# lmb-freiburg/hand3d

Measured on NVIDIA H100. Metric: images/sec full pipeline 320x320, higher is better.
Workload: dtype bf16 hi/lo split x3 MMA passes, fp32 accumulate (fp32 parity, 1e-3)

## Files before the change

### hand3d_b200/csrc/conv_wgmma.cu

```cuda
#include <cuda.h>

#include <algorithm>
#include <cstdlib>
#include <cstring>
#include <vector>

#include "common.cuh"
#include "split_fmt.cuh"
#include "wgmma_common.cuh"

namespace h3d {

namespace {

constexpr int BM = 128;
constexpr int BK = 64;
constexpr int kThreads = 384;
constexpr int kConsumerThreads = 256;
constexpr int A_TILE_BYTES = BM * BK * 2;
constexpr int STG_COLS = 64;
constexpr int STG_PITCH = STG_COLS + 1;
constexpr int STG_BYTES = BM * STG_PITCH * 4;
constexpr int kSmemBudget = 227 * 1024 - 2048 - STG_BYTES;

__host__ __device__ constexpr int stage_bytes(int BN, int PASSES) { return (PASSES >= 3 ? 2 : 1) * (A_TILE_BYTES + BN * BK * 2); }
__host__ __device__ constexpr int num_stages(int BN, int PASSES) {
    return kSmemBudget / stage_bytes(BN, PASSES) > 8 ? 8 : kSmemBudget / stage_bytes(BN, PASSES);
}
__host__ __device__ constexpr int smem_bytes(int BN, int PASSES) { return num_stages(BN, PASSES) * stage_bytes(BN, PASSES) + STG_BYTES + 2048; }

struct TcParams {
    const float* bias;
    uint16_t* y_hi; uint16_t* y_lo; uint8_t* y_l8; uint8_t* y_h8; int Cy_total, cy_off;
    float corr_scale;
    float* yf; int Cyf_total, cyf_off;
    int B, H, W, k, pad, cin_chunks;
    int TW, TH, TB, tiles_w, tiles_h, n_tiles, num_tiles;
    int n_valid;
    int pool;
    int chunk_kb;
    int leaky;
    int* err_flag;
};

template <int PASSES, bool FP16>
__device__ __forceinline__ void epilogue_store32(const TcParams& p, const float* a, int64_t pix, int n, bool valid) {
    float f[32];
    const float4* bp = reinterpret_cast<const float4*>(p.bias + n);
#pragma unroll
    for (int q = 0; q < 8; ++q) {
        const float4 bv = __ldg(bp + q);
        if (PASSES == 4) {
            f[4 * q + 0] = fmaf(a[4 * q + 0], p.corr_scale, bv.x);
            f[4 * q + 1] = fmaf(a[4 * q + 1], p.corr_scale, bv.y);
            f[4 * q + 2] = fmaf(a[4 * q + 2], p.corr_scale, bv.z);
            f[4 * q + 3] = fmaf(a[4 * q + 3], p.corr_scale, bv.w);
        } else {
            f[4 * q + 0] = a[4 * q + 0] + bv.x;
            f[4 * q + 1] = a[4 * q + 1] + bv.y;
            f[4 * q + 2] = a[4 * q + 2] + bv.z;
            f[4 * q + 3] = a[4 * q + 3] + bv.w;
        }
    }
    if (p.leaky) {
#pragma unroll
        for (int q = 0; q < 32; ++q) f[q] = fmaxf(f[q], kNegSlope * f[q]);
    }
    if (p.pool == 1) {
#pragma unroll
        for (int q = 0; q < 32; ++q) {
            f[q] = fmaxf(f[q], __shfl_xor_sync(0xFFFFFFFFu, f[q], 1));
            f[q] = fmaxf(f[q], __shfl_xor_sync(0xFFFFFFFFu, f[q], p.TW));
        }
    }
    if (!valid) return;
    if (n + 32 > p.n_valid) {
        const int cnt = p.n_valid - n;
        if (p.yf && cnt > 0) {
            float* dst = p.yf + pix * p.Cyf_total + p.cyf_off + n;
#pragma unroll
            for (int q = 0; q < 32; ++q)
                if (q < cnt) dst[q] = f[q];
        }
#pragma unroll
        for (int q = 0; q < 32; ++q)
            if (q >= cnt) f[q] = 0.f;
    } else if (p.yf) {
        if (((p.Cyf_total | p.cyf_off) & 3) == 0) {
            float4* dst = reinterpret_cast<float4*>(p.yf + pix * p.Cyf_total + p.cyf_off + n);
#pragma unroll
            for (int q = 0; q < 8; ++q) dst[q] = make_float4(f[4 * q], f[4 * q + 1], f[4 * q + 2], f[4 * q + 3]);
        } else {
            float* dst = p.yf + pix * p.Cyf_total + p.cyf_off + n;
#pragma unroll
            for (int q = 0; q < 32; ++q) dst[q] = f[q];
        }
    }
    if (p.y_hi) {
        const int64_t off = pix * p.Cy_total + p.cy_off + n;
        uint4* dh = reinterpret_cast<uint4*>(p.y_hi + off);
        uint4* dl = reinterpret_cast<uint4*>(p.y_lo + off);
#pragma unroll
        for (int g = 0; g < 4; ++g) {
            uint32_t hi[4], lo[4];
#pragma unroll
            for (int q = 0; q < 4; ++q) {
                float x0 = f[8 * g + 2 * q], x1 = f[8 * g + 2 * q + 1];
                if (PASSES == 4) {
                    x0 = fminf(fmaxf(x0 * kF8XMainScale, -65504.f), 65504.f);
                    x1 = fminf(fmaxf(x1 * kF8XMainScale, -65504.f), 65504.f);
                }
                hi[q] = pack_hi2<FP16>(x0, x1);
                if (PASSES == 3) {
                    const float2 r = unpack2<FP16>(hi[q]);
                    lo[q] = pack_hi2<FP16>(x0 - r.x, x1 - r.y);
                }
            }
            dh[g] = make_uint4(hi[0], hi[1], hi[2], hi[3]);
            if (PASSES == 3 && p.y_lo) dl[g] = make_uint4(lo[0], lo[1], lo[2], lo[3]);
        }
        if (PASSES == 4) {
            uint32_t l8[8], h8[8];
#pragma unroll
            for (int q = 0; q < 8; ++q) {
                uint32_t wl = 0, wh = 0;
#pragma unroll
                for (int e = 0; e < 4; ++e) {
                    const F8cPlanes pl = f32_to_f8c(f[4 * q + e]);
                    wl |= (uint32_t)pl.l8 << (8 * e); wh |= (uint32_t)pl.h8 << (8 * e);
                }
                l8[q] = wl; h8[q] = wh;
            }
            uint4* d8l = reinterpret_cast<uint4*>(p.y_l8 + off);
            uint4* d8h = reinterpret_cast<uint4*>(p.y_h8 + off);
            d8l[0] = make_uint4(l8[0], l8[1], l8[2], l8[3]); d8l[1] = make_uint4(l8[4], l8[5], l8[6], l8[7]);
            d8h[0] = make_uint4(h8[0], h8[1], h8[2], h8[3]); d8h[1] = make_uint4(h8[4], h8[5], h8[6], h8[7]);
        }
    }
}

template <int BN, int PASSES>
struct RingCfg {
    static constexpr int STAGES = num_stages(BN, PASSES);
    static constexpr int STAGE_BYTES = stage_bytes(BN, PASSES);
    static constexpr int B_TILE_BYTES = BN * BK * 2;
    static constexpr int A8_TILE_BYTES = BM * BK, B8_TILE_BYTES = BN * BK;
    static_assert(STAGES >= 3, "the consumers hold two stages while the producer refills a third");
};

template <int BN, int PASSES>
__device__ __forceinline__ void produce_kblock(Ring& r, const CUtensorMap* x_hi, const CUtensorMap* x_lo, const CUtensorMap* x_h8,
                                               const CUtensorMap* w_hi, const CUtensorMap* w_lo, const CUtensorMap* w_l8,
                                               int a0, int a1, int a2, int a3, int kcol, int n0, int* err_flag) {
    using C = RingCfg<BN, PASSES>;
    mbar_wait(&r.empty[r.stage], r.phase ^ 1, err_flag, 1);
    if (elect_one()) {
        uint8_t* st = r.base + r.stage * C::STAGE_BYTES;
        uint64_t* fb = &r.full[r.stage];
        mbar_expect_tx(fb, C::STAGE_BYTES);
        tma_load_4d(x_hi, st, fb, a0, a1, a2, a3);
        tma_load_2d(w_hi, st + (PASSES >= 3 ? 2 : 1) * A_TILE_BYTES, fb, kcol, n0);
        if (PASSES == 3) {
            tma_load_4d(x_lo, st + A_TILE_BYTES, fb, a0, a1, a2, a3);
            tma_load_2d(w_lo, st + 2 * A_TILE_BYTES + C::B_TILE_BYTES, fb, kcol, n0);
        }
        if (PASSES == 4) {
            tma_load_4d(x_lo, st + A_TILE_BYTES, fb, a0, a1, a2, a3);
            tma_load_4d(x_h8, st + A_TILE_BYTES + C::A8_TILE_BYTES, fb, a0, a1, a2, a3);
            tma_load_2d(w_lo, st + 2 * A_TILE_BYTES + C::B_TILE_BYTES, fb, kcol, n0);
            tma_load_2d(w_l8, st + 2 * A_TILE_BYTES + C::B_TILE_BYTES + C::B8_TILE_BYTES, fb, kcol, n0);
        }
    }
    __syncwarp();
    if (++r.stage == C::STAGES) { r.stage = 0; r.phase ^= 1; }
}

template <int BN, int PASSES, bool FP16>
__device__ __forceinline__ void mma_tile(Ring& r, int kblocks, int chunk_kb, float* racc, int wg, int lane, int* err_flag) {
    using C = RingCfg<BN, PASSES>;
    constexpr int NR = BN / 2;
    constexpr int NR8 = PASSES == 4 ? NR : 1;
    float acc[NR], acc8[NR8];
#pragma unroll
    for (int i = 0; i < NR; ++i) acc[i] = 0.f;
#pragma unroll
    for (int i = 0; i < NR8; ++i) acc8[i] = 0.f;
    for (int kb0 = 0; kb0 < kblocks; kb0 += chunk_kb) {
        const int kb1 = min(kblocks, kb0 + chunk_kb);
        int pend = -1;
        for (int kb = kb0; kb < kb1; ++kb) {
            mbar_wait(&r.full[r.stage], r.phase, err_flag, 3);
            const uint32_t sa = smem_u32(r.base + r.stage * C::STAGE_BYTES);
            const uint32_t a_rows = (uint32_t)wg * 64 * 128;
            const uint64_t a_hi = desc_sw128(sa + a_rows);
            const uint64_t a_lo = desc_sw128(sa + A_TILE_BYTES + a_rows);
            const uint64_t b_hi = desc_sw128(sa + (PASSES >= 3 ? 2 : 1) * A_TILE_BYTES);
            const uint64_t b_lo = desc_sw128(sa + 2 * A_TILE_BYTES + C::B_TILE_BYTES);
            fence_regs<NR>(acc);
            fence_regs<NR8>(acc8);
            wgmma_fence();
#pragma unroll
            for (int j = 0; j < BK / 16; ++j) {
                const uint64_t koff = (uint64_t)j * 2;
                mma16<BN, FP16>(acc, a_hi + koff, b_hi + koff, (uint32_t)((kb > kb0) | (j != 0)));
                if (PASSES == 3) {
                    mma16<BN, FP16>(acc, a_hi + koff, b_lo + koff, 1u);
                    mma16<BN, FP16>(acc, a_lo + koff, b_hi + koff, 1u);
                }
            }
            if (PASSES == 4) {
                const uint32_t a8_rows = (uint32_t)wg * 64 * 64;
                const uint64_t a_l8 = desc_sw64(sa + A_TILE_BYTES + a8_rows);
                const uint64_t a_h8 = desc_sw64(sa + A_TILE_BYTES + C::A8_TILE_BYTES + a8_rows);
                const uint64_t b_h8 = desc_sw64(sa + 2 * A_TILE_BYTES + C::B_TILE_BYTES);
                const uint64_t b_l8 = desc_sw64(sa + 2 * A_TILE_BYTES + C::B_TILE_BYTES + C::B8_TILE_BYTES);
#pragma unroll
                for (int j = 0; j < 2; ++j) {
                    const uint64_t koff = (uint64_t)j * 2;
                    mma8<BN>(acc8, a_l8 + koff, b_h8 + koff, (uint32_t)((kb > kb0) | (j != 0)));
                    mma8<BN>(acc8, a_h8 + koff, b_l8 + koff, 1u);
                }
            }
            wgmma_commit();
            fence_regs<NR>(acc);
            fence_regs<NR8>(acc8);
            wgmma_wait<1>();
            if (pend >= 0 && lane == 0) mbar_arrive(&r.empty[pend]);
            pend = r.stage;
            if (++r.stage == C::STAGES) { r.stage = 0; r.phase ^= 1; }
        }
        wgmma_wait<0>();
        if (lane == 0) mbar_arrive(&r.empty[pend]);
        fence_regs<NR>(acc);
        fence_regs<NR8>(acc8);
        if constexpr (PASSES == 4) {
#pragma unroll
            for (int i = 0; i < NR; ++i) acc[i] += acc8[i];
        }
        if (kb0 == 0) {
#pragma unroll
            for (int i = 0; i < NR; ++i) racc[i] = acc[i];
        } else {
#pragma unroll
            for (int i = 0; i < NR; ++i) racc[i] += acc[i];
        }
    }
}

template <int BN, int PASSES, bool FP16, class PixOf>
__device__ __forceinline__ void store_tile(const TcParams& p, const float* racc, float* stg, int ct, int n0, PixOf pix_of) {
    const int wg = ct >> 7, tt = ct & 127;
    const int r0 = wg * 64 + (tt >> 5) * 16 + ((tt & 31) >> 2);
    const int cq = 2 * (tt & 3);
    const int row = ct & 127, half = ct >> 7;
    int64_t pix; bool valid;
    pix_of(row, pix, valid);
#pragma unroll
    for (int rnd = 0; rnd < BN / STG_COLS; ++rnd) {
        named_bar_sync(1, kConsumerThreads);
#pragma unroll
        for (int j = 0; j < STG_COLS / 8; ++j) {
            const int jj = rnd * (STG_COLS / 8) + j, c = 8 * j + cq;
            stg[r0 * STG_PITCH + c] = racc[4 * jj];
            stg[r0 * STG_PITCH + c + 1] = racc[4 * jj + 1];
            stg[(r0 + 8) * STG_PITCH + c] = racc[4 * jj + 2];
            stg[(r0 + 8) * STG_PITCH + c + 1] = racc[4 * jj + 3];
        }
        named_bar_sync(1, kConsumerThreads);
        float f[32];
#pragma unroll
        for (int q = 0; q < 32; ++q) f[q] = stg[row * STG_PITCH + half * 32 + q];
        epilogue_store32<PASSES, FP16>(p, f, pix, n0 + rnd * STG_COLS + half * 32, valid);
    }
}

constexpr int kProducerRegs = 40, kConsumerRegs = 232;

template <int BN, int PASSES, bool FP16>
__global__ void __launch_bounds__(kThreads, 1)
conv_tc_kernel(const __grid_constant__ CUtensorMap map_x_hi, const __grid_constant__ CUtensorMap map_x_lo,
               const __grid_constant__ CUtensorMap map_w_hi, const __grid_constant__ CUtensorMap map_w_lo,
               const __grid_constant__ CUtensorMap map_x_h8, const __grid_constant__ CUtensorMap map_w_l8, const TcParams p) {
    using C = RingCfg<BN, PASSES>;
    static_assert(PASSES != 4 || FP16, "fp8-correction mode uses an fp16 main plane");
    static_assert(smem_bytes(BN, PASSES) <= 227 * 1024, "conv_tc_kernel: shared memory budget");

    extern __shared__ __align__(1024) uint8_t smem_raw[];
    uint8_t* smem = reinterpret_cast<uint8_t*>((reinterpret_cast<uintptr_t>(smem_raw) + 1023) & ~(uintptr_t)1023);
    float* stg = reinterpret_cast<float*>(smem + C::STAGES * C::STAGE_BYTES);
    uint64_t* bars = reinterpret_cast<uint64_t*>(smem + C::STAGES * C::STAGE_BYTES + STG_BYTES);
    Ring ring{smem, bars, bars + C::STAGES, 0, 0};

    const int warp = threadIdx.x >> 5, lane = threadIdx.x & 31;
    const int wg = __shfl_sync(0xFFFFFFFFu, (int)threadIdx.x / 128, 0);
    const int kblocks = p.k * p.k * p.cin_chunks;

    if (threadIdx.x == 0) {
        prefetch_tmap(&map_x_hi); prefetch_tmap(&map_w_hi);
        if (PASSES >= 3) { prefetch_tmap(&map_x_lo); prefetch_tmap(&map_w_lo); }
        if (PASSES == 4) { prefetch_tmap(&map_x_h8); prefetch_tmap(&map_w_l8); }
        for (int s = 0; s < C::STAGES; ++s) { mbar_init(&ring.full[s], 1); mbar_init(&ring.empty[s], kConsumerThreads / 32); }
        asm volatile("fence.mbarrier_init.release.cluster;" ::: "memory");
    }
    __syncthreads();
    pdl_launch_dependents();
    pdl_wait();

    if (wg == 0) {
        setmaxnreg_dec<kProducerRegs>();
        if (warp == 0) {
            for (int tile = blockIdx.x; tile < p.num_tiles; tile += gridDim.x) {
                const int nt = tile % p.n_tiles, mt = tile / p.n_tiles;
                const int tw = mt % p.tiles_w, th = (mt / p.tiles_w) % p.tiles_h, tb = mt / (p.tiles_w * p.tiles_h);
                const int w0 = tw * p.TW - p.pad, h0 = th * p.TH - p.pad, b0 = tb * p.TB, n0 = nt * BN;
                int kcol = 0;
                for (int kh = 0; kh < p.k; ++kh)
                    for (int kw = 0; kw < p.k; ++kw)
                        for (int cc = 0; cc < p.cin_chunks; ++cc, kcol += BK)
                            produce_kblock<BN, PASSES>(ring, &map_x_hi, &map_x_lo, &map_x_h8, &map_w_hi, &map_w_lo, &map_w_l8, cc * BK,
                                                       w0 + kw, h0 + kh, b0, kcol, n0, p.err_flag);
            }
        }
    } else {
        setmaxnreg_inc<kConsumerRegs>();
        const int ct = threadIdx.x - 128;
        float racc[BN / 2];
        for (int tile = blockIdx.x; tile < p.num_tiles; tile += gridDim.x) {
            const int nt = tile % p.n_tiles, mt = tile / p.n_tiles;
            const int tw = mt % p.tiles_w, th = (mt / p.tiles_w) % p.tiles_h, tb = mt / (p.tiles_w * p.tiles_h);
            mma_tile<BN, PASSES, FP16>(ring, kblocks, p.chunk_kb, racc, ct >> 7, lane, p.err_flag);
            store_tile<BN, PASSES, FP16>(p, racc, stg, ct, nt * BN, [&](int row, int64_t& pix, bool& valid) {
                const int w_l = row % p.TW, h_l = (row / p.TW) % p.TH, b_l = row / (p.TW * p.TH);
                const int w = tw * p.TW + w_l, h = th * p.TH + h_l, b = tb * p.TB + b_l;
                valid = (w < p.W) && (h < p.H) && (b < p.B);
                pix = ((int64_t)b * p.H + h) * p.W + w;
                if (p.pool) {
                    const int par = p.pool == 2 ? 1 : 0;
                    valid = valid && ((w & 1) == par) && ((h & 1) == par);
                    pix = ((int64_t)b * (p.H >> 1) + (h >> 1)) * (p.W >> 1) + (w >> 1);
                }
            });
        }
    }
}

constexpr int C3_TW = 16, C3_TH = 8;
constexpr int C3T_THREADS = 256;
constexpr int C3T_B_BYTES = 128 * BK * 2;
constexpr int C3T_PW = C3_TW + 2, C3T_PH = C3_TH + 2;
constexpr int C3T_PATCH_FLOATS = C3T_PH * C3T_PW * 3;
constexpr int C3T_SMEM = C3T_B_BYTES + 2 * A_TILE_BYTES + STG_BYTES + C3T_PATCH_FLOATS * 4 + 1024 ;

template <bool FP16>
__global__ void __launch_bounds__(C3T_THREADS, 2)
conv_c3_tc_kernel(const float* __restrict__ x, const float* __restrict__ w, const TcParams p) {
    extern __shared__ __align__(1024) uint8_t smem_raw[];
    uint8_t* smem = reinterpret_cast<uint8_t*>((reinterpret_cast<uintptr_t>(smem_raw) + 1023) & ~(uintptr_t)1023);
    uint8_t* bsm = smem;
    uint8_t* asm_ = smem + C3T_B_BYTES;
    float* stg = reinterpret_cast<float*>(asm_ + 2 * A_TILE_BYTES);
    float* patch = stg + BM * STG_PITCH;

    const int t = threadIdx.x, wg = t >> 7;
    if (t < 128) {
        const int co = t & 63;
        uint32_t pk[16];
#pragma unroll
        for (int k2 = 0; k2 < 16; ++k2) {
            float v0 = 0.f, v1 = 0.f;
            if (2 * k2 < 27) v0 = __ldg(w + (2 * k2) * 64 + co);
            if (2 * k2 + 1 < 27) v1 = __ldg(w + (2 * k2 + 1) * 64 + co);
            const uint32_t h = pack_hi2<FP16>(v0, v1);
            if (t < 64) pk[k2] = h;
            else { const float2 r = unpack2<FP16>(h); pk[k2] = pack_hi2<FP16>(v0 - r.x, v1 - r.y); }
        }
#pragma unroll
        for (int c = 0; c < 4; ++c)
            *reinterpret_cast<uint4*>(bsm + sw128_chunk(t, c)) = make_uint4(pk[4 * c], pk[4 * c + 1], pk[4 * c + 2], pk[4 * c + 3]);
    }
    pdl_launch_dependents();
    pdl_wait();

    const uint32_t sb = smem_u32(bsm), sa = smem_u32(asm_);
    const uint64_t b_hi = desc_sw128(sb), b_lo = desc_sw128(sb + 64 * 128);
    const uint64_t a_hi = desc_sw128(sa + wg * 64 * 128), a_lo = desc_sw128(sa + A_TILE_BYTES + wg * 64 * 128);
    for (int tile = blockIdx.x; tile < p.num_tiles; tile += gridDim.x) {
        const int tw = tile % p.tiles_w, th = (tile / p.tiles_w) % p.tiles_h, b = tile / (p.tiles_w * p.tiles_h);
        {
            const int x0 = tw * C3_TW - 1, y0 = th * C3_TH - 1;
            const float* xb = x + (int64_t)b * p.H * p.W * 3;
            for (int i = t; i < C3T_PATCH_FLOATS; i += C3T_THREADS) {
                const int r = i / (C3T_PW * 3), rem = i - r * (C3T_PW * 3);
                const int gy = y0 + r, gx = x0 + rem / 3;
                float v = 0.f;
                if (gy >= 0 && gy < p.H && gx >= 0 && gx < p.W) v = __ldg(xb + ((int64_t)gy * p.W + x0) * 3 + rem);
                patch[i] = v;
            }
        }
        __syncthreads();
        if (t < 128) {
            const int w_l = t % C3_TW, h_l = t / C3_TW;
            uint32_t hi[16], lo[16];
#pragma unroll
            for (int k2 = 0; k2 < 16; ++k2) {
                float v0 = 0.f, v1 = 0.f;
                if (2 * k2 < 27) { const int k = 2 * k2; v0 = patch[(h_l + k / 9) * (C3T_PW * 3) + w_l * 3 + (k % 9)]; }
                if (2 * k2 + 1 < 27) { const int k = 2 * k2 + 1; v1 = patch[(h_l + k / 9) * (C3T_PW * 3) + w_l * 3 + (k % 9)]; }
                hi[k2] = pack_hi2<FP16>(v0, v1);
                const float2 r = unpack2<FP16>(hi[k2]);
                lo[k2] = pack_hi2<FP16>(v0 - r.x, v1 - r.y);
            }
#pragma unroll
            for (int c = 0; c < 4; ++c) {
// ... 127 lines not shown
                    float c3[3];
                    const int kp = i / 3;
                    c3[0] = __ldcg(P.can + 63 * b + 3 * kp); c3[1] = __ldcg(P.can + 63 * b + 3 * kp + 1); c3[2] = __ldcg(P.can + 63 * b + 3 * kp + 2);
                    const int j = i - kp * 3;
                    const float cz = right ? -c3[2] : c3[2];
                    P.out[63 * b + i] = c3[0] * R[j] + c3[1] * R[3 + j] + cz * R[6 + j];
                }
            }
        }
    }
    cluster_sync_all();
}

}

typedef CUresult (*EncodeTiledFn)(CUtensorMap*, CUtensorMapDataType, cuuint32_t, void*, const cuuint64_t*, const cuuint64_t*,
                                  const cuuint32_t*, const cuuint32_t*, CUtensorMapInterleave, CUtensorMapSwizzle,
                                  CUtensorMapL2promotion, CUtensorMapFloatOOBfill);

EncodeTiledFn get_encode_fn() {
    static EncodeTiledFn fn = nullptr;
    if (fn) return fn;
    void* ptr = nullptr;
    cudaDriverEntryPointQueryResult qres;
    cudaError_t e = cudaGetDriverEntryPoint("cuTensorMapEncodeTiled", &ptr, cudaEnableDefault, &qres);
    if (e != cudaSuccess || qres != cudaDriverEntryPointSuccess || !ptr) {
        set_error("cuTensorMapEncodeTiled not available (%s)", cudaGetErrorString(e));
        return nullptr;
    }
    fn = reinterpret_cast<EncodeTiledFn>(ptr);
    return fn;
}

bool encode_act_map(CUtensorMap* m, const void* base, int C_total, int C_used, int W, int H, int B, int TW, int TH, int TB, int es) {
    EncodeTiledFn fn = get_encode_fn();
    if (!fn) return false;
    cuuint64_t dims[4] = {(cuuint64_t)C_used, (cuuint64_t)W, (cuuint64_t)H, (cuuint64_t)B};
    cuuint64_t strides[3] = {(cuuint64_t)C_total * es, (cuuint64_t)W * C_total * es, (cuuint64_t)H * W * C_total * es};
    cuuint32_t box[4] = {(cuuint32_t)BK, (cuuint32_t)TW, (cuuint32_t)TH, (cuuint32_t)TB};
    cuuint32_t estr[4] = {1, 1, 1, 1};
    CUresult r = fn(m, es == 2 ? CU_TENSOR_MAP_DATA_TYPE_UINT16 : CU_TENSOR_MAP_DATA_TYPE_UINT8, 4, const_cast<void*>(base), dims, strides,
                    box, estr, CU_TENSOR_MAP_INTERLEAVE_NONE, es == 2 ? CU_TENSOR_MAP_SWIZZLE_128B : CU_TENSOR_MAP_SWIZZLE_64B,
                    CU_TENSOR_MAP_L2_PROMOTION_L2_256B, CU_TENSOR_MAP_FLOAT_OOB_FILL_NONE);
    if (r != CUDA_SUCCESS) { set_error("cuTensorMapEncodeTiled(activations) failed: %d", (int)r); return false; }
    return true;
}

bool encode_w_map(CUtensorMap* m, const void* base, int Ktot, int Cout_pad, int BN, int es) {
    EncodeTiledFn fn = get_encode_fn();
    if (!fn) return false;
    cuuint64_t dims[2] = {(cuuint64_t)Ktot, (cuuint64_t)Cout_pad};
    cuuint64_t strides[1] = {(cuuint64_t)Ktot * es};
    cuuint32_t box[2] = {(cuuint32_t)BK, (cuuint32_t)BN};
    cuuint32_t estr[2] = {1, 1};
    CUresult r = fn(m, es == 2 ? CU_TENSOR_MAP_DATA_TYPE_UINT16 : CU_TENSOR_MAP_DATA_TYPE_UINT8, 2, const_cast<void*>(base), dims, strides,
                    box, estr, CU_TENSOR_MAP_INTERLEAVE_NONE, es == 2 ? CU_TENSOR_MAP_SWIZZLE_128B : CU_TENSOR_MAP_SWIZZLE_64B,
                    CU_TENSOR_MAP_L2_PROMOTION_L2_256B, CU_TENSOR_MAP_FLOAT_OOB_FILL_NONE);
    if (r != CUDA_SUCCESS) { set_error("cuTensorMapEncodeTiled(weights) failed: %d", (int)r); return false; }
    return true;
}

namespace {

void choose_tile(int B, int H, int W, int* TW, int* TH, int* TB, bool pool = false) {
    static const int cand[][3] = {{16, 8, 1}, {8, 16, 1}, {32, 4, 1}, {4, 32, 1}, {64, 2, 1}, {128, 1, 1}, {8, 8, 2},
                                  {16, 4, 2}, {4, 16, 2}, {8, 4, 4}, {4, 8, 4}, {4, 4, 8}, {8, 2, 8}, {2, 2, 32}, {1, 1, 128}};
    int64_t best = -1;
    for (auto& c : cand) {
        if (pool && !((c[0] % 2) == 0 && c[0] <= 16 && (c[1] % 2) == 0)) continue;
        const int64_t tiles = (int64_t)ceil_div(W, c[0]) * ceil_div(H, c[1]) * ceil_div(B, c[2]);
        if (best < 0 || tiles < best) { best = tiles; *TW = c[0]; *TH = c[1]; *TB = c[2]; }
    }
}

template <int BN, int PASSES, bool FP16>
int launch_inst(const TcConvPlan* pl, cudaStream_t s);

}

struct TcConvPlan {
    int device = 0;
    TcConvDesc d;
    CUtensorMap map_x_hi, map_x_lo, map_w_hi, map_w_lo, map_x_h8, map_w_l8;
    TcParams p;
    int BN, grid;
};

constexpr int kMaxDevices = 64;
static int current_device() { int dev = 0; if (cudaGetDevice(&dev) != cudaSuccess) { cudaGetLastError(); dev = 0; } return dev; }
int tc_num_sms() {
    static int n[kMaxDevices] = {};
    const int dev = current_device() % kMaxDevices;
    if (!n[dev]) {
        int v = 0;
        if (cudaDeviceGetAttribute(&v, cudaDevAttrMultiProcessorCount, dev) != cudaSuccess || v <= 0) { cudaGetLastError(); v = 132; }
        n[dev] = v;
    }
    return n[dev];
}
template <typename K>
static int smem_opt_in(K kernel, int bytes, bool* done ) {
    const int dev = current_device() % kMaxDevices;
    if (!done[dev]) {
        H3D_CUDA(cudaFuncSetAttribute(kernel, cudaFuncAttributeMaxDynamicSharedMemorySize, bytes));
        done[dev] = true;
    }
    return H3D_OK;
}

template <typename... KArgs, typename... Args>
static cudaError_t launch_pdl(void (*kernel)(KArgs...), dim3 grid, dim3 block, size_t smem, cudaStream_t s, Args&&... args) {
    cudaLaunchConfig_t cfg = {};
    cfg.gridDim = grid; cfg.blockDim = block; cfg.dynamicSmemBytes = smem; cfg.stream = s;
    cudaLaunchAttribute attr[1];
    attr[0].id = cudaLaunchAttributeProgrammaticStreamSerialization;
    attr[0].val.programmaticStreamSerializationAllowed = tc_tuning().pdl ? 1 : 0;
    cfg.attrs = attr; cfg.numAttrs = 1;
    return cudaLaunchKernelEx(&cfg, kernel, static_cast<KArgs>(args)...);
}

TcTuning& tc_tuning() {
    static TcTuning t = [] {
        TcTuning v;
        auto geti = [](const char* n, int d) { const char* e = getenv(n); return e ? atoi(e) : d; };
        v.two_cta = geti("H3D_TC_2CTA", -1);
        v.bn = geti("H3D_TC_BN", 0);
        v.c64 = geti("H3D_TC_C64", 1);
        v.c64x2 = geti("H3D_TC_C64X2", 1);
        v.pair128 = geti("H3D_TC_PAIR128", 1);
        v.stack = geti("H3D_TC_STACK", 1);
        v.chunk_kb = geti("H3D_TC_CHUNK_KB", 0);
        v.exp = geti("H3D_TC_EXP", 0);
        v.no_side_stream = geti("H3D_NO_SIDE_STREAM", 0);
        v.no_pool_fusion = geti("H3D_NO_POOL_FUSION", 0);
        v.lift_direct = geti("H3D_LIFT_DIRECT", 0);
        v.c3_ffma = geti("H3D_C3_FFMA", 0);
        v.c3_tma = geti("H3D_C3_TMA", 1);
        v.pdl = geti("H3D_PDL", 1);
        v.fc_chain = geti("H3D_FC_CHAIN", 1);
        v.c64_tma_out = geti("H3D_C64_TMA_OUT", 1);
        v.chain = geti("H3D_TC_CHAIN", 1);
        v.small_batch_split = geti("H3D_TC_SMALL_SPLIT", 1);
        v.fuse_c1 = geti("H3D_FUSE_C1", 1);
        v.no_seg_fusion = geti("H3D_NO_SEG_FUSION", 0);
        return v;
    }();
    return t;
}
int tc_set_tuning(const char* key, int value) {
    TcTuning& t = tc_tuning();
    const std::string k(key ? key : "");
    if (k == "tc_2cta") t.two_cta = value;
    else if (k == "tc_bn") t.bn = value;
    else if (k == "tc_c64") t.c64 = value;
    else if (k == "tc_c64x2") t.c64x2 = value;
    else if (k == "tc_pair128") t.pair128 = value;
    else if (k == "tc_stack") t.stack = value;
    else if (k == "tc_chunk_kb") t.chunk_kb = value;
    else if (k == "tc_exp") t.exp = value;
    else if (k == "no_side_stream") t.no_side_stream = value;
    else if (k == "no_pool_fusion") t.no_pool_fusion = value;
    else if (k == "lift_direct") t.lift_direct = value;
    else if (k == "c3_ffma") t.c3_ffma = value;
    else if (k == "c3_tma") t.c3_tma = value;
    else if (k == "pdl") t.pdl = value;
    else if (k == "fc_chain") t.fc_chain = value;
    else if (k == "c64_tma_out") t.c64_tma_out = value;
    else if (k == "tc_chain") t.chain = value;
    else if (k == "tc_small_split") t.small_batch_split = value;
    else if (k == "fuse_c1") t.fuse_c1 = value;
    else if (k == "no_seg_fusion") t.no_seg_fusion = value;
    else { set_error("h3d_set_tuning: unknown key '%s'", k.c_str()); return H3D_EINVAL; }
    return H3D_OK;
}

namespace {
template <int BN, int PASSES, bool FP16>
int launch_inst(const TcConvPlan* pl, cudaStream_t s) {
    constexpr int smem = smem_bytes(BN, PASSES);
    static bool attr[kMaxDevices] = {};
    if (int rc = smem_opt_in(conv_tc_kernel<BN, PASSES, FP16>, smem, attr)) return rc;
    H3D_CUDA(launch_pdl(conv_tc_kernel<BN, PASSES, FP16>, dim3(pl->grid), dim3(kThreads), smem, s, pl->map_x_hi, pl->map_x_lo, pl->map_w_hi,
                        pl->map_w_lo, pl->map_x_h8, pl->map_w_l8, pl->p));
    return H3D_OK;
}
}

TcConvPlan* tc_conv_plan_create(const TcConvDesc& d) {
    if (d.Cin_pad % BK != 0 || d.Cout_pad % 64 != 0 || (d.k != 1 && d.k != 3 && d.k != 5 && d.k != 7) || (d.passes != 1 && d.passes != 3 && d.passes != 4)) {
        set_error("tc_conv: unsupported geometry (Cin_pad=%d Cout_pad=%d k=%d passes=%d)", d.Cin_pad, d.Cout_pad, d.k, d.passes);
        return nullptr;
    }
    const bool padded_out = d.Cout % 32 != 0;
    if (d.y.hi && ((d.Cy_total % 8) || (d.cy_off % 8))) { set_error("tc_conv: split output channel offset/stride must be multiples of 8"); return nullptr; }
    if (d.yf && !padded_out && ((d.Cyf_total % 4) || (d.cyf_off % 4))) { set_error("tc_conv: fp32 output channel offset/stride must be multiples of 4"); return nullptr; }
    if (padded_out && d.pool == 1) { set_error("tc_conv: fused pooling needs Cout %% 32 == 0"); return nullptr; }
    if (d.pool < 0 || d.pool > 2) { set_error("tc_conv: pool mode must be 0 (none), 1 (max-pool) or 2 (stride 2)"); return nullptr; }
    if (d.pool == 2 && d.k < 3) { set_error("tc_conv: stride 2 needs k >= 3 (for k = 1 TF's 'SAME' samples the even pixels, not the odd ones)"); return nullptr; }
    if (d.c1_w) { set_error("tc_conv: conv1_1 is not fused into conv1_2 on sm_90a (tc_conv_can_fuse_first is false)"); return nullptr; }
    if (d.passes == 3 && (!d.x.lo || !d.w.lo)) { set_error("tc_conv: 3-pass mode needs lo planes"); return nullptr; }
    if (d.passes == 4 && (!d.x.l8 || !d.x.h8 || !d.w.l8 || !d.w.h8 || d.half != Half16::FP16 || d.corr_scale <= 0.f)) {
        set_error("tc_conv: fp8-correction mode needs fp16 + e4m3 l8/h8 planes for activations and weights and a correction scale");
        return nullptr;
    }
    if (d.passes == 4 && d.y.hi && (!d.y.l8 || !d.y.h8)) { set_error("tc_conv: fp8-correction mode needs l8/h8 output planes"); return nullptr; }
    if (d.passes == 4 && d.y.hi && ((d.Cy_total % 16) || (d.cy_off % 16))) { set_error("tc_conv: fp8 planes need 16-channel aligned offsets"); return nullptr; }
    if (d.pool && ((d.H | d.W) & 1)) { set_error("tc_conv: fused max-pool / stride 2 needs even H and W"); return nullptr; }
    TcConvPlan* pl = new TcConvPlan();
    pl->d = d;
    const TcTuning& tune = tc_tuning();
    int BN = d.Cout_pad % 128 == 0 ? 128 : 64;
    if ((int64_t)d.H * d.W <= 256) BN = 64;
    if ((tune.bn == 64 || tune.bn == 128) && d.Cout_pad % tune.bn == 0) BN = tune.bn;
    if (d.passes == 4) BN = 64;
    int TW, TH, TB;
    choose_tile(d.B, d.H, d.W, &TW, &TH, &TB, d.pool == 1);
    pl->BN = BN;
    pl->device = current_device();
    TcParams& p = pl->p;
    p.bias = d.bias;
    p.y_hi = d.y.hi; p.y_lo = d.y.lo; p.y_l8 = d.y.l8; p.y_h8 = d.y.h8; p.Cy_total = d.Cy_total; p.cy_off = d.cy_off;
    p.corr_scale = d.corr_scale;
    p.yf = d.yf; p.Cyf_total = d.Cyf_total; p.cyf_off = d.cyf_off;
    p.B = d.B; p.H = d.H; p.W = d.W; p.k = d.k; p.pad = d.k / 2; p.cin_chunks = d.Cin_pad / BK;
    p.TW = TW; p.TH = TH; p.TB = TB;
    p.tiles_w = ceil_div(d.W, TW); p.tiles_h = ceil_div(d.H, TH);
    p.n_tiles = d.Cout_pad / BN;
    p.num_tiles = p.tiles_w * p.tiles_h * ceil_div(d.B, TB) * p.n_tiles;
    p.leaky = d.leaky;
    p.n_valid = d.Cout;
    p.pool = d.pool;
    p.err_flag = d.err_flag;
    p.chunk_kb = d.passes >= 3 ? 9 : 27;
    if (tune.chunk_kb > 0) p.chunk_kb = tune.chunk_kb;
    pl->grid = std::min(p.num_tiles, tc_num_sms());
    const int Ktot = d.k * d.k * d.Cin_pad;
    bool ok = encode_act_map(&pl->map_x_hi, d.x.hi, d.Cin_total, d.Cin_pad, d.W, d.H, d.B, TW, TH, TB) &&
              encode_w_map(&pl->map_w_hi, d.w.hi, Ktot, d.Cout_pad, BN);
    if (ok && d.passes == 3)
        ok = encode_act_map(&pl->map_x_lo, d.x.lo, d.Cin_total, d.Cin_pad, d.W, d.H, d.B, TW, TH, TB) &&
             encode_w_map(&pl->map_w_lo, d.w.lo, Ktot, d.Cout_pad, BN);
    if (ok && d.passes == 4)
        ok = encode_act_map(&pl->map_x_lo, d.x.l8, d.Cin_total, d.Cin_pad, d.W, d.H, d.B, TW, TH, TB, 1) &&
             encode_act_map(&pl->map_x_h8, d.x.h8, d.Cin_total, d.Cin_pad, d.W, d.H, d.B, TW, TH, TB, 1) &&
             encode_w_map(&pl->map_w_lo, d.w.h8, Ktot, d.Cout_pad, BN, 1) &&
             encode_w_map(&pl->map_w_l8, d.w.l8, Ktot, d.Cout_pad, BN, 1);
    if (ok && d.passes == 1) { pl->map_x_lo = pl->map_x_hi; pl->map_w_lo = pl->map_w_hi; }
    if (ok && d.passes != 4) { pl->map_x_h8 = pl->map_x_hi; pl->map_w_l8 = pl->map_w_hi; }
    if (!ok) { delete pl; return nullptr; }
    return pl;
}

void tc_conv_plan_destroy(TcConvPlan* p) { delete p; }

bool tc_conv_plan_chainable(const TcConvPlan*) { return false; }
int tc_conv_plan_signal_target(const TcConvPlan* p) { return p->p.tiles_w * p->p.tiles_h * p->p.n_tiles; }
const TcConvDesc& tc_conv_plan_desc(const TcConvPlan* p) { return p->d; }
void tc_conv_plan_set_chain(TcConvPlan*, int*, const int*, int, int*) {}

int64_t tc_conv_flops(const TcConvPlan* p) {
    return 2ll * p->d.B * p->d.H * p->d.W * p->d.k * p->d.k * (int64_t)p->d.Cin_pad * p->d.Cout_pad;
}

bool tc_conv_can_fuse_first(int, int, int, int, int, int, int) { return false; }

int tc_conv_launch_image(const TcConvPlan*, const float*, cudaStream_t) {
    set_error("tc_conv_launch_image: conv1_1 is not fused into conv1_2 on sm_90a");
    return H3D_EINVAL;
}

int tc_conv_launch(const TcConvPlan* pl, cudaStream_t s) {
    const bool fp16 = pl->d.half == Half16::FP16;
    const int key = pl->BN * 10 + pl->d.passes;
#define CASE(BN_, P_)                                                                  \
    case BN_ * 10 + P_:                                                                \
        return fp16 ? launch_inst<BN_, P_, true>(pl, s) : launch_inst<BN_, P_, false>(pl, s);
    switch (key) {
        CASE(64, 1) CASE(64, 3) CASE(128, 1) CASE(128, 3)
        case 64 * 10 + 4: return launch_inst<64, 4, true>(pl, s);
    }
#undef CASE
    set_error("tc_conv: no kernel instance for BN=%d passes=%d", pl->BN, pl->d.passes);
    return H3D_EINVAL;
}

int launch_conv_c3_tc(const float* x, const float* w, const float* bias, Split y, int Cs_total, int cs_off, int B, int H, int W, int leaky,
                      Half16 half, cudaStream_t s, int* err_flag) {
    H3D_REQUIRE(x && w && bias && y.hi && !y.l8 && (Cs_total % 8) == 0 && (cs_off % 8) == 0, "conv_c3_tc: bad argument");
    TcParams p{};
    p.bias = bias;
    p.y_hi = y.hi; p.y_lo = y.lo; p.Cy_total = Cs_total; p.cy_off = cs_off;
    p.corr_scale = 1.f;
    p.B = B; p.H = H; p.W = W; p.k = 3; p.pad = 1; p.cin_chunks = 1;
    p.TW = C3_TW; p.TH = C3_TH; p.TB = 1;
    p.tiles_w = ceil_div(W, C3_TW); p.tiles_h = ceil_div(H, C3_TH); p.n_tiles = 1;
    p.num_tiles = p.tiles_w * p.tiles_h * B;
    p.n_valid = 64; p.pool = 0; p.chunk_kb = 1; p.leaky = leaky; p.err_flag = err_flag;
    const int grid = std::min(p.num_tiles, 2 * tc_num_sms());
    static bool attr_h[kMaxDevices] = {}, attr_b[kMaxDevices] = {};
    if (int rc = smem_opt_in(conv_c3_tc_kernel<true>, C3T_SMEM, attr_h)) return rc;
    if (int rc = smem_opt_in(conv_c3_tc_kernel<false>, C3T_SMEM, attr_b)) return rc;
    if (half == Half16::FP16) H3D_CUDA(launch_pdl(conv_c3_tc_kernel<true>, dim3(grid), dim3(C3T_THREADS), (size_t)C3T_SMEM, s, x, w, p));
    else H3D_CUDA(launch_pdl(conv_c3_tc_kernel<false>, dim3(grid), dim3(C3T_THREADS), (size_t)C3T_SMEM, s, x, w, p));
    return H3D_OK;
}

struct FcChainPlan { FcChainParams P; Half16 half; int grid; };

FcChainPlan* fc_chain_plan_create(const FcChainDesc* chains, int num_chains, int B, Half16 half, const float* can, const float* uxyz,
                                  unsigned int* counter, int* err_flag) {
    if (num_chains < 1 || num_chains > 2 || B < 1) { set_error("fc_chain: bad geometry"); return nullptr; }
    FcChainPlan* pl = new FcChainPlan();
    memset(&pl->P, 0, sizeof(pl->P));
    pl->half = half; pl->grid = num_chains * kFcCluster;
    FcChainParams& P = pl->P;
    P.num_chains = num_chains; P.B = B; P.can = can; P.uxyz = uxyz; P.counter = counter; P.err_flag = err_flag;
    for (int c = 0; c < num_chains; ++c) {
        const FcChainDesc& cd = chains[c];
        if (cd.num_layers < 1 || cd.num_layers > kFcMaxLayers) { set_error("fc_chain: 1..4 layers per chain"); delete pl; return nullptr; }
        P.chain[c].num_layers = cd.num_layers;
        for (int l = 0; l < cd.num_layers; ++l) {
            const FcLayerDesc& d = cd.layer[l];
            FcLayer& L = P.chain[c].layer[l];
            const int Kpad = (int)align_up(d.in_features, BK);
            if (!d.x.hi || !d.x.lo || !d.w.hi || !d.w.lo || d.out_pad % 64 || d.x_stride < Kpad || (d.y.hi && (d.y_stride % 8))) {
                set_error("fc_chain: bad layer %d of chain %d", l, c); delete pl; return nullptr;
            }
            bool ok = encode_act_map(&L.map_x_hi, d.x.hi, d.x_stride, Kpad, 1, 1, B, 1, 1, BM) &&
                      encode_act_map(&L.map_x_lo, d.x.lo, d.x_stride, Kpad, 1, 1, B, 1, 1, BM) &&
                      encode_w_map(&L.map_w_hi, d.w.hi, Kpad, d.out_pad, 64) && encode_w_map(&L.map_w_lo, d.w.lo, Kpad, d.out_pad, 64);
            if (!ok) { delete pl; return nullptr; }
// ... 31 lines not shown
```

Baseline: 1014.

## Share taller activation halo tiles across kernel rows with split A/B rings

The implicit-GEMM conv producer now loads one activation tile covering g consecutive kernel rows (TH+g-1 rows) per (kw, cin chunk) and reuses it for g k-blocks by offsetting the smem row. Weights stream through a separate B ring. This cuts repeated TMA activation loads for overlapping kh taps, lowering L2/smem fill traffic. The cost is more complex ring bookkeeping, tail tensor maps, and runtime-sized smem, which may leave fewer pipeline stages.

```diff
diff --git a/hand3d_b200/csrc/conv_wgmma.cu b/hand3d_b200/csrc/conv_wgmma.cu
--- a/hand3d_b200/csrc/conv_wgmma.cu
+++ b/hand3d_b200/csrc/conv_wgmma.cu
@@ -21,7 +21,8 @@
 constexpr int STG_COLS = 64;
 constexpr int STG_PITCH = STG_COLS + 1;
 constexpr int STG_BYTES = BM * STG_PITCH * 4;
-constexpr int kSmemBudget = 227 * 1024 - 2048 - STG_BYTES;
+constexpr int kSmemMax = 227 * 1024;
+constexpr int kSmemBudget = kSmemMax - 2048 - STG_BYTES;
 
 __host__ __device__ constexpr int stage_bytes(int BN, int PASSES) { return (PASSES >= 3 ? 2 : 1) * (A_TILE_BYTES + BN * BK * 2); }
 __host__ __device__ constexpr int num_stages(int BN, int PASSES) {
@@ -41,6 +42,7 @@
     int chunk_kb;
     int leaky;
     int* err_flag;
+    int g, a_stages, b_stages, a_plane, a_tail_bytes;
 };
 
 template <int PASSES, bool FP16>
@@ -147,6 +149,52 @@
     static constexpr int A8_TILE_BYTES = BM * BK, B8_TILE_BYTES = BN * BK;
     static_assert(STAGES >= 3, "the consumers hold two stages while the producer refills a third");
 };
+
+__device__ __forceinline__ void ring_next(Ring& r, int stages) { if (++r.stage == stages) { r.stage = 0; r.phase ^= 1; } }
+
+template <int BN, int PASSES, bool FP16>
+__device__ __forceinline__ void mma_kblock(float* acc, float* acc8, uint32_t a_hi, uint32_t a_lo, uint32_t a_l8, uint32_t a_h8, uint32_t sb,
+                                           bool first) {
+    constexpr int B_TILE_BYTES = BN * BK * 2, B8_TILE_BYTES = BN * BK;
+    const uint64_t da_hi = desc_sw128(a_hi), da_lo = desc_sw128(a_lo);
+    const uint64_t b_hi = desc_sw128(sb);
+    const uint64_t b_lo = desc_sw128(sb + B_TILE_BYTES);
+#pragma unroll
+    for (int j = 0; j < BK / 16; ++j) {
+        const uint64_t koff = (uint64_t)j * 2;
+        mma16<BN, FP16>(acc, da_hi + koff, b_hi + koff, (uint32_t)(!first | (j != 0)));
+        if (PASSES == 3) {
+            mma16<BN, FP16>(acc, da_hi + koff, b_lo + koff, 1u);
+            mma16<BN, FP16>(acc, da_lo + koff, b_hi + koff, 1u);
+        }
+    }
+    if (PASSES == 4) {
+        const uint64_t da_l8 = desc_sw64(a_l8), da_h8 = desc_sw64(a_h8);
+        const uint64_t b_h8 = desc_sw64(sb + B_TILE_BYTES);
+        const uint64_t b_l8 = desc_sw64(sb + B_TILE_BYTES + B8_TILE_BYTES);
+#pragma unroll
+        for (int j = 0; j < 2; ++j) {
+            const uint64_t koff = (uint64_t)j * 2;
+            mma8<BN>(acc8, da_l8 + koff, b_h8 + koff, (uint32_t)(!first | (j != 0)));
+            mma8<BN>(acc8, da_h8 + koff, b_l8 + koff, 1u);
+        }
+    }
+}
+
+template <int NR, int NR8, int PASSES>
+__device__ __forceinline__ void fold_chunk(float* racc, float* acc, const float* acc8, bool first_chunk) {
+    if constexpr (PASSES == 4) {
+#pragma unroll
+        for (int i = 0; i < NR; ++i) acc[i] += acc8[i];
+    }
+    if (first_chunk) {
+#pragma unroll
+        for (int i = 0; i < NR; ++i) racc[i] = acc[i];
+    } else {
+#pragma unroll
+        for (int i = 0; i < NR; ++i) racc[i] += acc[i];
+    }
+}
 
 template <int BN, int PASSES>
 __device__ __forceinline__ void produce_kblock(Ring& r, const CUtensorMap* x_hi, const CUtensorMap* x_lo, const CUtensorMap* x_h8,
@@ -191,59 +239,130 @@
         for (int kb = kb0; kb < kb1; ++kb) {
             mbar_wait(&r.full[r.stage], r.phase, err_flag, 3);
             const uint32_t sa = smem_u32(r.base + r.stage * C::STAGE_BYTES);
-            const uint32_t a_rows = (uint32_t)wg * 64 * 128;
-            const uint64_t a_hi = desc_sw128(sa + a_rows);
-            const uint64_t a_lo = desc_sw128(sa + A_TILE_BYTES + a_rows);
-            const uint64_t b_hi = desc_sw128(sa + (PASSES >= 3 ? 2 : 1) * A_TILE_BYTES);
-            const uint64_t b_lo = desc_sw128(sa + 2 * A_TILE_BYTES + C::B_TILE_BYTES);
+            const uint32_t a_rows = (uint32_t)wg * 64 * 128, a8_rows = (uint32_t)wg * 64 * 64;
             fence_regs<NR>(acc);
             fence_regs<NR8>(acc8);
             wgmma_fence();
-#pragma unroll
-            for (int j = 0; j < BK / 16; ++j) {
-                const uint64_t koff = (uint64_t)j * 2;
-                mma16<BN, FP16>(acc, a_hi + koff, b_hi + koff, (uint32_t)((kb > kb0) | (j != 0)));
-                if (PASSES == 3) {
-                    mma16<BN, FP16>(acc, a_hi + koff, b_lo + koff, 1u);
-                    mma16<BN, FP16>(acc, a_lo + koff, b_hi + koff, 1u);
-                }
-            }
-            if (PASSES == 4) {
-                const uint32_t a8_rows = (uint32_t)wg * 64 * 64;
-                const uint64_t a_l8 = desc_sw64(sa + A_TILE_BYTES + a8_rows);
-                const uint64_t a_h8 = desc_sw64(sa + A_TILE_BYTES + C::A8_TILE_BYTES + a8_rows);
-                const uint64_t b_h8 = desc_sw64(sa + 2 * A_TILE_BYTES + C::B_TILE_BYTES);
-                const uint64_t b_l8 = desc_sw64(sa + 2 * A_TILE_BYTES + C::B_TILE_BYTES + C::B8_TILE_BYTES);
-#pragma unroll
-                for (int j = 0; j < 2; ++j) {
-                    const uint64_t koff = (uint64_t)j * 2;
-                    mma8<BN>(acc8, a_l8 + koff, b_h8 + koff, (uint32_t)((kb > kb0) | (j != 0)));
-                    mma8<BN>(acc8, a_h8 + koff, b_l8 + koff, 1u);
-                }
-            }
+            mma_kblock<BN, PASSES, FP16>(acc, acc8, sa + a_rows, sa + A_TILE_BYTES + a_rows, sa + A_TILE_BYTES + a8_rows,
+                                         sa + A_TILE_BYTES + C::A8_TILE_BYTES + a8_rows, sa + (PASSES >= 3 ? 2 : 1) * A_TILE_BYTES, kb == kb0);
             wgmma_commit();
             fence_regs<NR>(acc);
             fence_regs<NR8>(acc8);
             wgmma_wait<1>();
             if (pend >= 0 && lane == 0) mbar_arrive(&r.empty[pend]);
             pend = r.stage;
-            if (++r.stage == C::STAGES) { r.stage = 0; r.phase ^= 1; }
+            ring_next(r, C::STAGES);
         }
         wgmma_wait<0>();
         if (lane == 0) mbar_arrive(&r.empty[pend]);
         fence_regs<NR>(acc);
         fence_regs<NR8>(acc8);
-        if constexpr (PASSES == 4) {
-#pragma unroll
-            for (int i = 0; i < NR; ++i) acc[i] += acc8[i];
-        }
-        if (kb0 == 0) {
-#pragma unroll
-            for (int i = 0; i < NR; ++i) racc[i] = acc[i];
-        } else {
-#pragma unroll
-            for (int i = 0; i < NR; ++i) racc[i] += acc[i];
-        }
+        fold_chunk<NR, NR8, PASSES>(racc, acc, acc8, kb0 == 0);
+    }
+}
+
+constexpr int kMaxRing = 8;
+
+template <int BN, int PASSES>
+__device__ __forceinline__ constexpr int b_stage_bytes() { return (PASSES >= 3 ? 2 : 1) * BN * BK * 2; }
+
+struct ConvRing { Ring a, b; };
+struct ConvMaps { const CUtensorMap *x_hi, *x_lo, *x_h8, *xt_hi, *xt_lo, *xt_h8, *w_hi, *w_lo, *w_l8; };
+
+template <int BN, int PASSES>
+__device__ __forceinline__ void produce_conv_tile(ConvRing& r, const ConvMaps& m, const TcParams& p, int w0, int h0, int b0, int n0) {
+    constexpr int B_TILE_BYTES = BN * BK * 2, B8_TILE_BYTES = BN * BK;
+    const int a_entry = (PASSES >= 3 ? 2 : 1) * p.a_plane;
+    for (int kw = 0; kw < p.k; ++kw)
+        for (int cc = 0; cc < p.cin_chunks; ++cc)
+            for (int kh0 = 0; kh0 < p.k; kh0 += p.g) {
+                const bool tail = kh0 + p.g > p.k;
+                mbar_wait(&r.a.empty[r.a.stage], r.a.phase ^ 1, p.err_flag, 1);
+                if (elect_one()) {
+                    uint8_t* st = r.a.base + r.a.stage * a_entry;
+                    uint64_t* fb = &r.a.full[r.a.stage];
+                    mbar_expect_tx(fb, tail ? p.a_tail_bytes : a_entry);
+                    tma_load_4d(tail ? m.xt_hi : m.x_hi, st, fb, cc * BK, w0 + kw, h0 + kh0, b0);
+                    if (PASSES >= 3) tma_load_4d(tail ? m.xt_lo : m.x_lo, st + p.a_plane, fb, cc * BK, w0 + kw, h0 + kh0, b0);
+                    if (PASSES == 4) tma_load_4d(tail ? m.xt_h8 : m.x_h8, st + p.a_plane + p.a_plane / 2, fb, cc * BK, w0 + kw, h0 + kh0, b0);
+                }
+                __syncwarp();
+                ring_next(r.a, p.a_stages);
+                const int kh1 = min(p.k, kh0 + p.g);
+                for (int kh = kh0; kh < kh1; ++kh) {
+                    const int kcol = ((kh * p.k + kw) * p.cin_chunks + cc) * BK;
+                    mbar_wait(&r.b.empty[r.b.stage], r.b.phase ^ 1, p.err_flag, 1);
+                    if (elect_one()) {
+                        uint8_t* st = r.b.base + r.b.stage * b_stage_bytes<BN, PASSES>();
+                        uint64_t* fb = &r.b.full[r.b.stage];
+                        mbar_expect_tx(fb, b_stage_bytes<BN, PASSES>());
+                        tma_load_2d(m.w_hi, st, fb, kcol, n0);
+                        if (PASSES >= 3) tma_load_2d(m.w_lo, st + B_TILE_BYTES, fb, kcol, n0);
+                        if (PASSES == 4) tma_load_2d(m.w_l8, st + B_TILE_BYTES + B8_TILE_BYTES, fb, kcol, n0);
+                    }
+                    __syncwarp();
+                    ring_next(r.b, p.b_stages);
+                }
+            }
+}
+
+template <int BN, int PASSES, bool FP16>
+__device__ __forceinline__ void mma_conv_tile(ConvRing& r, const TcParams& p, float* racc, int wg, int lane) {
+    constexpr int NR = BN / 2;
+    constexpr int NR8 = PASSES == 4 ? NR : 1;
+    const int a_entry = (PASSES >= 3 ? 2 : 1) * p.a_plane;
+    const int kblocks = p.k * p.k * p.cin_chunks;
+    float acc[NR], acc8[NR8];
+#pragma unroll
+    for (int i = 0; i < NR; ++i) acc[i] = 0.f;
+#pragma unroll
+    for (int i = 0; i < NR8; ++i) acc8[i] = 0.f;
+    int kh = 0, kh0 = 0, kh1 = min(p.k, p.g);
+    uint32_t row0 = 0;
+    for (int kb0 = 0; kb0 < kblocks; kb0 += p.chunk_kb) {
+        const int kb1 = min(kblocks, kb0 + p.chunk_kb);
+        int pend_a = -1, pend_b = -1;
+        for (int kb = kb0; kb < kb1; ++kb) {
+            if (kh == kh0) {
+                mbar_wait(&r.a.full[r.a.stage], r.a.phase, p.err_flag, 3);
+                row0 = (uint32_t)wg * (p.TB == 2 ? p.TW * (p.TH + kh1 - kh0 - 1) : 64);
+            }
+            mbar_wait(&r.b.full[r.b.stage], r.b.phase, p.err_flag, 3);
+            const uint32_t sa = smem_u32(r.a.base + r.a.stage * a_entry);
+            const uint32_t row = row0 + (uint32_t)((kh - kh0) * p.TW);
+            fence_regs<NR>(acc);
+            fence_regs<NR8>(acc8);
+            wgmma_fence();
+            mma_kblock<BN, PASSES, FP16>(acc, acc8, sa + row * 128, sa + p.a_plane + row * 128, sa + p.a_plane + row * 64,
+                                         sa + p.a_plane + p.a_plane / 2 + row * 64,
+                                         smem_u32(r.b.base + r.b.stage * b_stage_bytes<BN, PASSES>()), kb == kb0);
+            wgmma_commit();
+            fence_regs<NR>(acc);
+            fence_regs<NR8>(acc8);
+            wgmma_wait<1>();
+            if (lane == 0) {
+                if (pend_b >= 0) mbar_arrive(&r.b.empty[pend_b]);
+                if (pend_a >= 0) mbar_arrive(&r.a.empty[pend_a]);
+            }
+            pend_b = r.b.stage;
+            ring_next(r.b, p.b_stages);
+            pend_a = -1;
+            if (++kh == kh1) {
+                pend_a = r.a.stage;
+                ring_next(r.a, p.a_stages);
+                if (kh == p.k) kh = 0;
+                kh0 = kh;
+                kh1 = min(p.k, kh0 + p.g);
+            }
+        }
+        wgmma_wait<0>();
+        if (lane == 0) {
+            mbar_arrive(&r.b.empty[pend_b]);
+            if (pend_a >= 0) mbar_arrive(&r.a.empty[pend_a]);
+        }
+        fence_regs<NR>(acc);
+        fence_regs<NR8>(acc8);
+        fold_chunk<NR, NR8, PASSES>(racc, acc, acc8, kb0 == 0);
     }
 }
 
@@ -280,26 +399,32 @@
 __global__ void __launch_bounds__(kThreads, 1)
 conv_tc_kernel(const __grid_constant__ CUtensorMap map_x_hi, const __grid_constant__ CUtensorMap map_x_lo,
                const __grid_constant__ CUtensorMap map_w_hi, const __grid_constant__ CUtensorMap map_w_lo,
-               const __grid_constant__ CUtensorMap map_x_h8, const __grid_constant__ CUtensorMap map_w_l8, const TcParams p) {
-    using C = RingCfg<BN, PASSES>;
+               const __grid_constant__ CUtensorMap map_x_h8, const __grid_constant__ CUtensorMap map_w_l8,
+               const __grid_constant__ CUtensorMap map_xt_hi, const __grid_constant__ CUtensorMap map_xt_lo,
+               const __grid_constant__ CUtensorMap map_xt_h8, const TcParams p) {
     static_assert(PASSES != 4 || FP16, "fp8-correction mode uses an fp16 main plane");
-    static_assert(smem_bytes(BN, PASSES) <= 227 * 1024, "conv_tc_kernel: shared memory budget");
 
     extern __shared__ __align__(1024) uint8_t smem_raw[];
     uint8_t* smem = reinterpret_cast<uint8_t*>((reinterpret_cast<uintptr_t>(smem_raw) + 1023) & ~(uintptr_t)1023);
-    float* stg = reinterpret_cast<float*>(smem + C::STAGES * C::STAGE_BYTES);
-    uint64_t* bars = reinterpret_cast<uint64_t*>(smem + C::STAGES * C::STAGE_BYTES + STG_BYTES);
-    Ring ring{smem, bars, bars + C::STAGES, 0, 0};
+    uint8_t* b_base = smem + p.a_stages * (PASSES >= 3 ? 2 : 1) * p.a_plane;
+    float* stg = reinterpret_cast<float*>(b_base + p.b_stages * b_stage_bytes<BN, PASSES>());
+    uint64_t* bars = reinterpret_cast<uint64_t*>(reinterpret_cast<uint8_t*>(stg) + STG_BYTES);
+    ConvRing ring{{smem, bars, bars + kMaxRing, 0, 0}, {b_base, bars + 2 * kMaxRing, bars + 3 * kMaxRing, 0, 0}};
 
     const int warp = threadIdx.x >> 5, lane = threadIdx.x & 31;
     const int wg = __shfl_sync(0xFFFFFFFFu, (int)threadIdx.x / 128, 0);
-    const int kblocks = p.k * p.k * p.cin_chunks;
 
     if (threadIdx.x == 0) {
         prefetch_tmap(&map_x_hi); prefetch_tmap(&map_w_hi);
         if (PASSES >= 3) { prefetch_tmap(&map_x_lo); prefetch_tmap(&map_w_lo); }
         if (PASSES == 4) { prefetch_tmap(&map_x_h8); prefetch_tmap(&map_w_l8); }
-        for (int s = 0; s < C::STAGES; ++s) { mbar_init(&ring.full[s], 1); mbar_init(&ring.empty[s], kConsumerThreads / 32); }
+        if (p.k % p.g) {
+            prefetch_tmap(&map_xt_hi);
+            if (PASSES >= 3) prefetch_tmap(&map_xt_lo);
+            if (PASSES == 4) prefetch_tmap(&map_xt_h8);
+        }
+        for (int s = 0; s < p.a_stages; ++s) { mbar_init(&ring.a.full[s], 1); mbar_init(&ring.a.empty[s], kConsumerThreads / 32); }
+        for (int s = 0; s < p.b_stages; ++s) { mbar_init(&ring.b.full[s], 1); mbar_init(&ring.b.empty[s], kConsumerThreads / 32); }
         asm volatile("fence.mbarrier_init.release.cluster;" ::: "memory");
     }
     __syncthreads();
@@ -309,16 +434,11 @@
     if (wg == 0) {
         setmaxnreg_dec<kProducerRegs>();
         if (warp == 0) {
+            const ConvMaps maps{&map_x_hi, &map_x_lo, &map_x_h8, &map_xt_hi, &map_xt_lo, &map_xt_h8, &map_w_hi, &map_w_lo, &map_w_l8};
             for (int tile = blockIdx.x; tile < p.num_tiles; tile += gridDim.x) {
                 const int nt = tile % p.n_tiles, mt = tile / p.n_tiles;
                 const int tw = mt % p.tiles_w, th = (mt / p.tiles_w) % p.tiles_h, tb = mt / (p.tiles_w * p.tiles_h);
-                const int w0 = tw * p.TW - p.pad, h0 = th * p.TH - p.pad, b0 = tb * p.TB, n0 = nt * BN;
-                int kcol = 0;
-                for (int kh = 0; kh < p.k; ++kh)
-                    for (int kw = 0; kw < p.k; ++kw)
-                        for (int cc = 0; cc < p.cin_chunks; ++cc, kcol += BK)
-                            produce_kblock<BN, PASSES>(ring, &map_x_hi, &map_x_lo, &map_x_h8, &map_w_hi, &map_w_lo, &map_w_l8, cc * BK,
-                                                       w0 + kw, h0 + kh, b0, kcol, n0, p.err_flag);
+                produce_conv_tile<BN, PASSES>(ring, maps, p, tw * p.TW - p.pad, th * p.TH - p.pad, tb * p.TB, nt * BN);
             }
         }
     } else {
@@ -328,7 +448,7 @@
         for (int tile = blockIdx.x; tile < p.num_tiles; tile += gridDim.x) {
             const int nt = tile % p.n_tiles, mt = tile / p.n_tiles;
             const int tw = mt % p.tiles_w, th = (mt / p.tiles_w) % p.tiles_h, tb = mt / (p.tiles_w * p.tiles_h);
-            mma_tile<BN, PASSES, FP16>(ring, kblocks, p.chunk_kb, racc, ct >> 7, lane, p.err_flag);
+            mma_conv_tile<BN, PASSES, FP16>(ring, p, racc, ct >> 7, lane);
             store_tile<BN, PASSES, FP16>(p, racc, stg, ct, nt * BN, [&](int row, int64_t& pix, bool& valid) {
                 const int w_l = row % p.TW, h_l = (row / p.TW) % p.TH, b_l = row / (p.TW * p.TH);
                 const int w = tw * p.TW + w_l, h = th * p.TH + h_l, b = tb * p.TB + b_l;
@@ -622,8 +742,9 @@
     int device = 0;
     TcConvDesc d;
     CUtensorMap map_x_hi, map_x_lo, map_w_hi, map_w_lo, map_x_h8, map_w_l8;
+    CUtensorMap map_xt_hi, map_xt_lo, map_xt_h8;
     TcParams p;
-    int BN, grid;
+    int BN, grid, smem;
 };
 
 constexpr int kMaxDevices = 64;
@@ -717,12 +838,29 @@
 namespace {
 template <int BN, int PASSES, bool FP16>
 int launch_inst(const TcConvPlan* pl, cudaStream_t s) {
-    constexpr int smem = smem_bytes(BN, PASSES);
     static bool attr[kMaxDevices] = {};
-    if (int rc = smem_opt_in(conv_tc_kernel<BN, PASSES, FP16>, smem, attr)) return rc;
-    H3D_CUDA(launch_pdl(conv_tc_kernel<BN, PASSES, FP16>, dim3(pl->grid), dim3(kThreads), smem, s, pl->map_x_hi, pl->map_x_lo, pl->map_w_hi,
-                        pl->map_w_lo, pl->map_x_h8, pl->map_w_l8, pl->p));
+    if (int rc = smem_opt_in(conv_tc_kernel<BN, PASSES, FP16>, kSmemMax, attr)) return rc;
+    H3D_CUDA(launch_pdl(conv_tc_kernel<BN, PASSES, FP16>, dim3(pl->grid), dim3(kThreads), (size_t)pl->smem, s, pl->map_x_hi, pl->map_x_lo,
+                        pl->map_w_hi, pl->map_w_lo, pl->map_x_h8, pl->map_w_l8, pl->map_xt_hi, pl->map_xt_lo, pl->map_xt_h8, pl->p));
     return H3D_OK;
+}
+
+void plan_rings(int BN, int passes, int k, int TW, int TH, int TB, TcParams& p) {
+    const int planes = passes >= 3 ? 2 : 1;
+    const int b_bytes = planes * BN * BK * 2;
+    auto a_plane = [&](int g) { return TW * (TH + g - 1) * TB * BK * 2; };
+    const int S = std::min(kMaxRing, kSmemBudget / (planes * a_plane(1) + b_bytes));
+    const bool rows_ok = TW % 8 == 0 && (TB == 1 || (TB == 2 && TW * TH == 64));
+    int g = 1;
+    for (int c = k; rows_ok && c > 1; --c)
+        if (2 * planes * a_plane(c) + S * b_bytes <= kSmemBudget) { g = c; break; }
+    p.g = g;
+    p.a_plane = a_plane(g);
+    p.a_stages = g == 1 ? S : 2;
+    p.b_stages = g == 1 ? S : std::min(kMaxRing, (kSmemBudget - 2 * planes * p.a_plane) / b_bytes);
+    if (g > 1)
+        p.a_stages = std::min(kMaxRing, (kSmemBudget - p.b_stages * b_bytes) / (planes * p.a_plane));
+    p.a_tail_bytes = planes * a_plane(k % g ? k % g : g);
 }
 }
 
@@ -774,19 +912,23 @@
     p.chunk_kb = d.passes >= 3 ? 9 : 27;
     if (tune.chunk_kb > 0) p.chunk_kb = tune.chunk_kb;
     pl->grid = std::min(p.num_tiles, tc_num_sms());
+    plan_rings(BN, d.passes, d.k, TW, TH, TB, p);
+    pl->smem = p.a_stages * (d.passes >= 3 ? 2 : 1) * p.a_plane + p.b_stages * (d.passes >= 3 ? 2 : 1) * BN * BK * 2 + STG_BYTES + 2048;
     const int Ktot = d.k * d.k * d.Cin_pad;
-    bool ok = encode_act_map(&pl->map_x_hi, d.x.hi, d.Cin_total, d.Cin_pad, d.W, d.H, d.B, TW, TH, TB) &&
-              encode_w_map(&pl->map_w_hi, d.w.hi, Ktot, d.Cout_pad, BN);
+    const int bh = TH + p.g - 1, bh_t = TH + (d.k % p.g ? d.k % p.g : p.g) - 1;
+    auto act_maps = [&](CUtensorMap* m, CUtensorMap* mt, const void* x, int es) {
+        return encode_act_map(m, x, d.Cin_total, d.Cin_pad, d.W, d.H, d.B, TW, bh, TB, es) &&
+               encode_act_map(mt, x, d.Cin_total, d.Cin_pad, d.W, d.H, d.B, TW, bh_t, TB, es);
+    };
+    bool ok = act_maps(&pl->map_x_hi, &pl->map_xt_hi, d.x.hi, 2) && encode_w_map(&pl->map_w_hi, d.w.hi, Ktot, d.Cout_pad, BN);
     if (ok && d.passes == 3)
-        ok = encode_act_map(&pl->map_x_lo, d.x.lo, d.Cin_total, d.Cin_pad, d.W, d.H, d.B, TW, TH, TB) &&
-             encode_w_map(&pl->map_w_lo, d.w.lo, Ktot, d.Cout_pad, BN);
+        ok = act_maps(&pl->map_x_lo, &pl->map_xt_lo, d.x.lo, 2) && encode_w_map(&pl->map_w_lo, d.w.lo, Ktot, d.Cout_pad, BN);
     if (ok && d.passes == 4)
-        ok = encode_act_map(&pl->map_x_lo, d.x.l8, d.Cin_total, d.Cin_pad, d.W, d.H, d.B, TW, TH, TB, 1) &&
-             encode_act_map(&pl->map_x_h8, d.x.h8, d.Cin_total, d.Cin_pad, d.W, d.H, d.B, TW, TH, TB, 1) &&
+        ok = act_maps(&pl->map_x_lo, &pl->map_xt_lo, d.x.l8, 1) && act_maps(&pl->map_x_h8, &pl->map_xt_h8, d.x.h8, 1) &&
              encode_w_map(&pl->map_w_lo, d.w.h8, Ktot, d.Cout_pad, BN, 1) &&
              encode_w_map(&pl->map_w_l8, d.w.l8, Ktot, d.Cout_pad, BN, 1);
-    if (ok && d.passes == 1) { pl->map_x_lo = pl->map_x_hi; pl->map_w_lo = pl->map_w_hi; }
-    if (ok && d.passes != 4) { pl->map_x_h8 = pl->map_x_hi; pl->map_w_l8 = pl->map_w_hi; }
+    if (ok && d.passes == 1) { pl->map_x_lo = pl->map_x_hi; pl->map_xt_lo = pl->map_xt_hi; pl->map_w_lo = pl->map_w_hi; }
+    if (ok && d.passes != 4) { pl->map_x_h8 = pl->map_x_hi; pl->map_xt_h8 = pl->map_xt_hi; pl->map_w_l8 = pl->map_w_hi; }
     if (!ok) { delete pl; return nullptr; }
     return pl;
 }
```

New measurement: 1037, median of 6. 1.02x the previous value.
